# h-brough/TUNA

Hardware: AMD Instinct MI355X
Metric: Fock builds/sec (J+K from the HBM-resident ERI tensor, one density) + SCF wall time (higher is better)
Workload: dtype f64

## Files before the change

tuna_amd/csrc/tf_device.hip:

```cpp
#include <hip/hip_runtime.h>

#include <algorithm>
#include <chrono>
#include <cmath>
#include <cstddef>
#include <cstdio>
#include <cstdlib>
#include <array>
#include <cstring>
#include <condition_variable>
#include <dlfcn.h>
#include <atomic>
#include <map>
#include <memory>
#include <mutex>
#include <thread>
#include <numeric>
#include <string>
#include <vector>

#include "../../include/tunafock.h"
#include "tf_internal.h"
#include "tf_kernels.hip.h"
#include "tf_jkpacked.hip.h"
// ... 2381 lines not shown
    HIPCHK(ctx, e);
    return TF_OK;
}


extern "C++" {
template <int ND>
static int jk_packed_pass(tf_ctx *ctx, hipStream_t st, double *const *dDout, bool cd = false)
{
    const BLayout &L = ctx->bl;
    const int N = ctx->N, NW = L.NW;
    const size_t nn = (size_t)N * N, npr = (size_t)L.NPtot, nrows = (size_t)std::max<long long>(1, ctx->n_rows);
    const tf_ctx::JKTables &T = ctx->jkt[ND - 1];
    const size_t ng = (size_t)std::max(1, T.n_groups);
    JKStrides S{};
    const int MP = ctx->hl.MP;
    S.KS = ctx->hl.KS; S.MP = MP;
    S.planeJd = nrows * NW; S.planeI = ng * N; S.planeJ = nrows * N;
    S.P = nn; S.Pp = npr; S.y = (size_t)T.ypart_len; S.Jd = MP * S.planeJd;
    S.DIc = MP * S.planeI; S.DIr = ng * (size_t)L.RS; S.DJc = MP * S.planeJ; S.DJr = nrows * (size_t)L.RS;
    const size_t per_g = (size_t)N * MP + L.RS;
    double *const pJrow = cd ? ctx->cd_Jrow : ctx->d_Jrow;
    double *const pY = cd ? ctx->cd_ypart + (ND == 2 ? (size_t)std::max<long long>(0, ctx->jkt[0].ypart_len) : 0) : ctx->d_ypart;
    const JKTask *const tasks = cd ? T.d_tasks_cd : T.d_tasks;
    const int n_tasks = cd ? T.n_tasks_cd : T.n_tasks;
    const int *const bucket = cd ? T.bucket_cd : T.bucket;
    double *DI0 = (cd ? ctx->cd_DI : ctx->d_DI) + (ND == 2 ? (size_t)std::max(1, ctx->jkt[0].n_groups) * per_g : 0);
    double *DJ0 = (cd ? ctx->cd_DJ : ctx->d_DJ) + (ND == 2 ? nrows * per_g : 0);
    double *DIc = DI0, *DIr = DI0 + ND * S.DIc, *DJc = DJ0, *DJr = DJ0 + ND * S.DJc;
    if (n_tasks > 0) {
        hipEvent_t ev_after = nullptr;
        if (ctx->prof_jk) {
            if (ctx->prof_used + 2 > ctx->prof_ev.size()) {
                hipEvent_t a, b;
                if (hipEventCreate(&a) == hipSuccess && hipEventCreate(&b) == hipSuccess) { ctx->prof_ev.push_back(a); ctx->prof_ev.push_back(b); }
            }
            if (ctx->prof_used + 2 <= ctx->prof_ev.size()) {
                (void)hipEventRecord(ctx->prof_ev[ctx->prof_used], st);
                ev_after = ctx->prof_ev[ctx->prof_used + 1];
                ctx->prof_used += 2;
            }
        }
        static const bool serial = getenv("TF_JK_SERIAL") != nullptr;
        int n_launch = 0;
        for (int b = 0; b < 3; ++b) n_launch += (bucket[b + 1] > bucket[b] && (TF_JKP_W >> b) >= 1) ? 1 : 0;
        static const int one_launch_below = getenv("TF_JK_ONE_LAUNCH") ? atoi(getenv("TF_JK_ONE_LAUNCH")) : 12000;
        const bool full_supers = T.n_supers > 0 && ctx->n_rows >= 24LL * T.n_supers;
        const bool one_launch = n_launch > 1 && n_tasks < one_launch_below && (ctx->world == 1 || full_supers);
        const bool fork = !serial && !one_launch && ctx->have_streams && n_launch > 1;
        if (fork) (void)hipEventRecord(ctx->sev[0], st);
        int side = 0;
        bool first = true;
        if (one_launch)
            hipLaunchKernelGGL((jk_packed_kernel<ND>), dim3((unsigned)n_tasks), dim3(64 * TF_JKP_W), 0, st, ctx->d_eri, T.d_groups,
                               T.d_supers, tasks, L, L.kinfo, ctx->d_Psym, ctx->d_Pp, pJrow, pY, DIc, DIr, DJc, DJr, S);
        for (int b = 0; b < 3 && !one_launch; ++b) {
            const int t0 = bucket[b], t1 = bucket[b + 1];
            if (!(t1 > t0 && (TF_JKP_W >> b) >= 1)) continue;
            hipStream_t ls = st;
            if (fork && !first) {
                ++side;
                ls = ctx->streams[side];
                (void)hipStreamWaitEvent(ls, ctx->sev[0], 0);
            }
            first = false;
            hipLaunchKernelGGL((jk_packed_kernel<ND>), dim3((unsigned)(t1 - t0)), dim3(64 * (TF_JKP_W >> b)), 0, ls, ctx->d_eri, T.d_groups,
                               T.d_supers, tasks + t0, L, L.kinfo, ctx->d_Psym, ctx->d_Pp, pJrow, pY, DIc, DIr, DJc, DJr, S);
            if (ls != st) {
                (void)hipEventRecord(ctx->sev[side], ls);
                (void)hipStreamWaitEvent(st, ctx->sev[side], 0);
            }
        }
        if (ev_after) (void)hipEventRecord(ev_after, st);
    }
    JKReduce R{};
    R.ypart = pY; R.sy = S.y; R.supers = T.d_supers; R.MC = ctx->hl.MC; R.MP = MP; R.planeI = S.planeI; R.planeJ = S.planeJ; R.nseg = T.nseg; R.jp = T.jp;
    R.Jt = ctx->d_Jt; R.sJt = (size_t)T.nseg * npr;
    R.DIc = DIc; R.sDIc = S.DIc; R.DIr = DIr; R.sDIr = S.DIr; R.DJc = DJc; R.sDJc = S.DJc; R.DJr = DJr; R.sDJr = S.DJr;
    R.gfirst = T.d_gfirst; R.jptr = ctx->d_jptr; R.jrows = ctx->d_jrows; R.row_ij = ctx->d_row_ij; R.xorder = ctx->d_xorder;
    for (int d = 0; d < ND; ++d) R.D[d] = dDout[d];
    { static const int jkr_dbg = getenv("TF_JKR_DBG") ? atoi(getenv("TF_JKR_DBG")) : 0; R.dbg = jkr_dbg; }
    const unsigned nblk = (unsigned)ND * ((unsigned)N * ((N + 127) / 128) + (unsigned)T.jp.bfirst[4] * T.nseg);
    hipLaunchKernelGGL(jk_reduce_kernel, dim3(nblk), dim3(TF_JKR_THREADS), 0, st, R, L);
    return TF_OK;
}
}

static int launch_jk_packed(tf_ctx *ctx, int nd, const double *const *dP, double *const *dJ, double *const *dK, hipStream_t st,
                            const int *nonsym)
{
    const BLayout &L = ctx->bl;
    const int N = ctx->N, NW = L.NW;
    const size_t nn = (size_t)N * N, npr = (size_t)L.NPtot, nrows = (size_t)std::max<long long>(1, ctx->n_rows);
    const dim3 gN((N * N + 255) / 256), b256(256);
    static const bool no_fuse = getenv("TF_JK_NOFUSE") != nullptr;
    bool cd = false;
    {
        static const bool cd_off = getenv("TF_JK_CLASS_DIAGONAL") && getenv("TF_JK_CLASS_DIAGONAL")[0] == '0';
        bool any_general = false;
        for (int d = 0; d < nd; ++d) any_general = any_general || (nonsym && nonsym[d]);
        static const int cd_nmin = getenv("TF_JK_CD_NMIN") ? atoi(getenv("TF_JK_CD_NMIN")) : 160;
        if (ctx->jk_try_class_diagonal && !cd_off && !any_general && N >= cd_nmin && ctx->jkt[0].n_tasks_cd < ctx->jkt[0].n_tasks) {
            if (!ctx->d_cdflag) HIPCHK(ctx, tf_malloc((void **)&ctx->d_cdflag, 2 * sizeof(unsigned long long)));
            cd = true;
            for (int d = 0; d < nd && cd; ++d) {
                HIPCHK(ctx, hipMemsetAsync(ctx->d_cdflag, 0, 2 * sizeof(unsigned long long), st));
                hipLaunchKernelGGL(class_cross_max_kernel, dim3((unsigned)N), dim3(256), 0, st, dP[d], L, ctx->d_cdflag);
                double h[2] = {0.0, 1.0};
                HIPCHK(ctx, hipMemcpyAsync(h, ctx->d_cdflag, sizeof(h), hipMemcpyDeviceToHost, st));
                HIPCHK(ctx, hipStreamSynchronize(st));
                cd = std::isfinite(h[0]) && h[0] < 1e299 && h[1] <= 1e-14 * h[0];
            }
            if (cd && !ctx->cd_Jrow) {
                double **bufs[4] = {&ctx->cd_Jrow, &ctx->cd_ypart, &ctx->cd_DI, &ctx->cd_DJ};
                for (int q = 0; q < 4; ++q) {
                    if (tf_malloc((void **)bufs[q], ctx->cd_bytes[q]) != hipSuccess) {
                        (void)hipGetLastError();
                        for (int u = 0; u < q; ++u) { (void)tf_free(*bufs[u]); *bufs[u] = nullptr; }
                        cd = false;
// ... 901 lines not shown
```

tuna_amd/csrc/tf_jkpacked.hip.h:

```cpp
#pragma once
#include <hip/hip_runtime.h>
#include "tf_layout.hip.h"

#include "tf_packed.h"
#ifndef TF_JKP_OCC4
#define TF_JKP_OCC4 3
#endif
#ifndef TF_JKP_STAGES
#define TF_JKP_STAGES 2
#endif


#ifndef TF_TRI_PAD
#define TF_TRI_PAD 16
#endif
__host__ __device__ inline long long tri_off(long long k)
{
    const long long q = k / TF_TRI_PAD, r = k % TF_TRI_PAD;
    return TF_TRI_PAD * (TF_TRI_PAD * q * (q + 1) / 2 + r * (q + 1));
}
__host__ __device__ inline long long packed_row_len(long long i, long long j) { return (tri_off(i) + j + TF_TRI_PAD) & ~(long long)(TF_TRI_PAD - 1); }

#define TF_JKP_KB 4

__device__ __forceinline__ double ld_stream(const double *p) { return __builtin_nontemporal_load(p); }

__device__ __forceinline__ __amdgpu_buffer_rsrc_t buf_rsrc(const void *base)
{
    return __builtin_amdgcn_make_buffer_rsrc(const_cast<void *>(base), 0, 0x7fffffff, 0x00020000);
}
template <int AUX>
__device__ __forceinline__ double2 buf_load2(__amdgpu_buffer_rsrc_t rs, unsigned lane_off, unsigned uniform_off)
{
    return __builtin_bit_cast(double2, __builtin_amdgcn_raw_buffer_load_b128(rs, (int)lane_off, (int)uniform_off, AUX));
}
template <int AUX>
__device__ __forceinline__ void buf_store2(__amdgpu_buffer_rsrc_t rs, unsigned lane_off, unsigned uniform_off, double2 v)
{
    typedef unsigned u4_t __attribute__((ext_vector_type(4)));
    __builtin_amdgcn_raw_buffer_store_b128(__builtin_bit_cast(u4_t, v), rs, (int)lane_off, (int)uniform_off, AUX);
}

typedef unsigned tf_u2 __attribute__((ext_vector_type(2)));

__device__ __forceinline__ double pair_step32(double a, double b)
{
    const tf_u2 lo = __builtin_amdgcn_permlane32_swap((unsigned)__double2loint(a), (unsigned)__double2loint(b), false, false);
    const tf_u2 hi = __builtin_amdgcn_permlane32_swap((unsigned)__double2hiint(a), (unsigned)__double2hiint(b), false, false);
    return __hiloint2double((int)hi.x, (int)lo.x) + __hiloint2double((int)hi.y, (int)lo.y);
}

__device__ __forceinline__ double pair_step16(double a, double b)
{
    const tf_u2 lo = __builtin_amdgcn_permlane16_swap((unsigned)__double2loint(a), (unsigned)__double2loint(b), false, false);
    const tf_u2 hi = __builtin_amdgcn_permlane16_swap((unsigned)__double2hiint(a), (unsigned)__double2hiint(b), false, false);
    return __hiloint2double((int)hi.x, (int)lo.x) + __hiloint2double((int)hi.y, (int)lo.y);
}

template <int CTRL, int BANK>
__device__ __forceinline__ double dpp_merge(double old, double src)
{
    const int lo = __builtin_amdgcn_update_dpp(__double2loint(old), __double2loint(src), CTRL, 0xF, BANK, false);
    const int hi = __builtin_amdgcn_update_dpp(__double2hiint(old), __double2hiint(src), CTRL, 0xF, BANK, false);
    return __hiloint2double(hi, lo);
}

#define TF_DPP_ROR8 0x128
#define TF_DPP_HALF_MIRROR 0x141
#define TF_DPP_QUAD_IDENT 0xE4
#define TF_DPP_QUAD_XOR1 0xB1
#define TF_DPP_QUAD_XOR2 0x4E

__device__ __forceinline__ double pair_step8(double a, double b)
{
    double recv = dpp_merge<TF_DPP_ROR8, 0x3>(a, a);
    recv = dpp_merge<TF_DPP_ROR8, 0xC>(recv, b);
// ... 97 lines not shown
}
__device__ __forceinline__ double quarter_sum8(const double (&v)[8])
{
    const double w0 = pair_step8(v[0], v[4]), w1 = pair_step8(v[1], v[5]), w2 = pair_step8(v[2], v[6]), w3 = pair_step8(v[3], v[7]);
    const double u0 = pair_step4(w0, w2), u1 = pair_step4(w1, w3);
    double t = pair_step2(u0, u1, (__lane_id() & 2u) != 0u);
    t += dpp_merge<TF_DPP_QUAD_XOR1, 0xF>(t, t);
    return t;
}
__device__ __forceinline__ double quarter_sum1(double t)
{
    t += dpp_merge<TF_DPP_ROR8, 0xF>(t, t);
    return sum8(t);
}
#if TF_JKP_GPW == 4
#define TF_JKP_VSH 1
__device__ __forceinline__ double group_sum8(const double (&v)[8]) { return quarter_sum8(v); }
__device__ __forceinline__ double group_sum1(double t) { return quarter_sum1(t); }
__device__ __forceinline__ double across_groups(double t) { t = pair_step32(t, t); return pair_step16(t, t); }
#else
#define TF_JKP_VSH 2
__device__ __forceinline__ double group_sum8(const double (&v)[8]) { return half_sum8(v); }
__device__ __forceinline__ double group_sum1(double t) { return half_sum1(t); }
__device__ __forceinline__ double across_groups(double t) { return pair_step32(t, t); }
#endif
#define TF_JKP_VMASK ((1 << TF_JKP_VSH) - 1)

#define TF_BUF_OOB 0x80000000u
template <int AUX>
__device__ __forceinline__ void buf_store1(__amdgpu_buffer_rsrc_t rs, unsigned lane_off, unsigned uniform_off, double v)
{
    typedef unsigned u2_t __attribute__((ext_vector_type(2)));
    __builtin_amdgcn_raw_buffer_store_b64(__builtin_bit_cast(u2_t, v), rs, (int)lane_off, (int)uniform_off, AUX);
}
template <int AUX>
__device__ __forceinline__ double buf_load1(__amdgpu_buffer_rsrc_t rs, unsigned lane_off, unsigned uniform_off)
{
    return __builtin_bit_cast(double, __builtin_amdgcn_raw_buffer_load_b64(rs, (int)lane_off, (int)uniform_off, AUX));
}

struct JKWave {
    const double *Tb, *X, *Pp;
    const KInfo *kinfo;
    long long NPtot;
    int N, i;
    int kI0, c0, lam0, width, cm;
    int sec;
    __amdgpu_buffer_rsrc_t rt;
    int rp;
    double *yg, *DIr, *DJr;
    size_t RS, ystride, dstrideI, dstrideJ;
};

template <int ND>
struct JKLane {
    int h, q, lam, lI;
    int nr, lamj0, r0, g;
    unsigned xrow;
    unsigned gb, unr, p0;
    unsigned djoff, dioff;
    double ppij[JKShape<ND>::VR];
    double2 pil[ND], pjl[JKShape<ND>::VR];
    double2 colI[ND], colJ[JKShape<ND>::VR];
};

enum { JKP_DIAG = 1, JKP_FULL = 2 };

template <int ND>
struct JKLoad { double2 m[JKShape<ND>::RB], pp[ND]; int cnt; };

template <int ND, bool ALLR, int MODE>
__device__ __forceinline__ void jkp_load(JKLoad<ND> &L, const JKLane<ND> &C, const JKWave &U, int kap)
{
    constexpr int RB = JKShape<ND>::RB;
    const KInfo ki = U.kinfo[kap];
    const int pc = (ki.cnt + TF_SEG_PAD - 1) & ~(TF_SEG_PAD - 1);
    L.cnt = ki.cnt;
    const bool v = (MODE == JKP_FULL) || C.lam < ki.cnt;
    const __amdgpu_buffer_rsrc_t rt = U.rt;
    const unsigned seg = __umul24(C.p0, (unsigned)pc) + __umul24(C.unr, (unsigned)(U.sec + ki.offA)) + C.gb;
    const unsigned dsel = 8u * seg;
#ifdef TF_ABL_ALLVALID
    const unsigned voff = 16u * (unsigned)C.q + dsel;
#define TF_ABL_ROWOK(r) true
#else
    const unsigned voff = v ? 16u * (unsigned)C.q + dsel : TF_BUF_OOB;
#define TF_ABL_ROWOK(r) (ALLR || (r) < C.nr)
#endif
#pragma unroll
#ifdef TF_ABL_NOTENSOR
    for (int r = 0; r < RB; ++r) L.m[r] = make_double2(C.ppij[r] + (double)kap, C.ppij[r] - (double)voff);
#else
    for (int r = 0; r < RB; ++r) L.m[r] = buf_load2<2>(rt, TF_ABL_ROWOK(r) ? voff : TF_BUF_OOB, 8u * (unsigned)(r * pc));
#endif
    const long long bk = (long long)ki.offA + U.lam0;
#pragma unroll
    for (int d = 0; d < ND; ++d) L.pp[d] = buf_load2<0>(buf_rsrc(U.Pp + d * U.NPtot + bk), v ? 16u * (unsigned)C.q : TF_BUF_OOB, 0u);
}

template <int ND>
__device__ __forceinline__ void jkp_row1(const JKLane<ND> &C, const JKLoad<ND> &L, double (&jd)[JKShape<ND>::VR],
                                         double (&rJ)[JKShape<ND>::VR], double (&rI)[ND], double2 (&jt)[ND])
{
    constexpr int RB = JKShape<ND>::RB;
#pragma unroll
    for (int d = 0; d < ND; ++d) {
        jt[d] = make_double2(0.0, 0.0);
        rI[d] = 0.0;
#pragma unroll
        for (int r = 0; r < RB; ++r) {
            const int v = d * RB + r;
            const double2 m = L.m[r];
            jd[v] += m.x * L.pp[d].x + m.y * L.pp[d].y;
            jt[d].x += m.x * C.ppij[v]; jt[d].y += m.y * C.ppij[v];
            const double2 pj = C.pjl[v];
            rI[d] += m.x * pj.x + m.y * pj.y;
            rJ[v] = m.x * C.pil[d].x + m.y * C.pil[d].y;
        }
    }
}

template <int ND, int MODE>
__device__ __forceinline__ void jkp_row2(JKLane<ND> &C, const JKLoad<ND> &L, const JKWave &U, const double (&pjk)[JKShape<ND>::VR], const double (&pik)[ND])
{
    constexpr int RB = JKShape<ND>::RB;
    const int lim = L.cnt - U.cm;
    const double o0 = (MODE == JKP_FULL || C.lam < lim) ? 1.0 : 0.0, o1 = (MODE == JKP_FULL || C.lam + 1 < lim) ? 1.0 : 0.0;
#pragma unroll
    for (int r = 0; r < RB; ++r) {
        const double mx = (MODE == JKP_FULL) ? L.m[r].x : L.m[r].x * o0, my = (MODE == JKP_FULL) ? L.m[r].y : L.m[r].y * o1;
#pragma unroll
        for (int d = 0; d < ND; ++d) {
            const int v = d * RB + r;
            C.colI[d].x += mx * pjk[v]; C.colI[d].y += my * pjk[v];
            C.colJ[v].x += mx * pik[d]; C.colJ[v].y += my * pik[d];
        }
    }
}

template <int ND, bool ALLR>
__device__ __forceinline__ void jkp_p_k(const JKLane<ND> &C, const JKWave &U, int kI, double (&pjk)[JKShape<ND>::VR], double (&pik)[ND])
{
    constexpr int RB = JKShape<ND>::RB;
#pragma unroll
    for (int d = 0; d < ND; ++d) {
        const double *Pd = U.X + (size_t)d * U.N * U.N;
        const __amdgpu_buffer_rsrc_t rx = buf_rsrc(Pd);
#pragma unroll
#ifdef TF_ABL_NOPJK
        for (int r = 0; r < RB; ++r) pjk[d * RB + r] = C.ppij[d * RB + r];
#else
        for (int r = 0; r < RB; ++r) pjk[d * RB + r] = buf_load1<0>(rx, (ALLR || r < C.nr) ? C.xrow : TF_BUF_OOB, 8u * (unsigned)(r * U.N + kI));
#endif
        pik[d] = Pd[(size_t)U.i * U.N + kI];
    }
}

template <int ND>
__device__ __forceinline__ void jkp_last(JKLane<ND> &C, const JKWave &U, const double (&pjk)[JKShape<ND>::VR], const double (&pik)[ND],
                                         double (&jd)[JKShape<ND>::VR], double (&rJ)[JKShape<ND>::VR], double (&rI)[ND], double2 (&jt2)[ND])
{
    constexpr int RB = JKShape<ND>::RB;
    const int i = U.i, lamlast = C.lamj0 + C.nr - 1;
    const KInfo kiL = U.kinfo[i - U.kI0];
    const long long bk = kiL.offA;
    const int pc = (kiL.cnt + TF_SEG_PAD - 1) & ~(TF_SEG_PAD - 1);
    const double *Tk = U.Tb + ((long long)C.gb + (long long)C.unr * (U.sec + kiL.offA) + (long long)C.p0 * pc);
#pragma unroll
    for (int d = 0; d < ND; ++d) { rI[d] = 0.0; jt2[d] = make_double2(0.0, 0.0); }
#pragma unroll
    for (int v = 0; v < JKShape<ND>::VR; ++v) rJ[v] = 0.0;
#pragma unroll
    for (int e = 0; e < 2; ++e) {
        const int lam = C.lam + e;
        const bool valid = lam <= lamlast;
        double mrow[RB];
#pragma unroll
        for (int r = 0; r < RB; ++r) mrow[r] = (r < C.nr && lam <= C.lamj0 + r) ? ld_stream(Tk + r * pc + lam) : 0.0;
#pragma unroll
        for (int d = 0; d < ND; ++d) {
            const double pp = valid ? U.Pp[d * U.NPtot + bk + lam] : 0.0;
            const double pil = e ? C.pil[d].y : C.pil[d].x;
            double jt = 0.0, cI = 0.0;
#pragma unroll
            for (int r = 0; r < RB; ++r) {
                const int v = d * RB + r;
                const double mr = mrow[r];
                const bool diag = (lam == C.lamj0 + r);
                jd[v] += mr * pp;
                jt += diag ? 0.0 : mr * C.ppij[v];
                const double mk = diag ? 0.5 * mr : mr;
                rI[d] += mk * (e ? C.pjl[v].y : C.pjl[v].x);
                rJ[v] += mk * pil;
                const double mc = (C.lI + e != i) ? mk : 0.0;
                cI += mc * pjk[v];
                if (e) C.colJ[v].y += mc * pik[d]; else C.colJ[v].x += mc * pik[d];
            }
            if (e) { C.colI[d].y += cI; jt2[d].y = jt; } else { C.colI[d].x += cI; jt2[d].x = jt; }
        }
    }
}

template <int ND, bool ALLR>
__device__ __forceinline__ void jkp_row_sums(const JKLane<ND> &C, const JKWave &U, int kap, double (&rJ)[JKShape<ND>::VR], const double (&rI)[ND])
{
    constexpr int VR = JKShape<ND>::VR, RB = JKShape<ND>::RB;
    const int v = (C.q >> TF_JKP_VSH) & 7;
    const bool first = (C.q & TF_JKP_VMASK) == 0;
    if constexpr (VR == 8) {
        const double tJ = group_sum8(rJ);
        const int d = v / RB, r = v - d * RB;
        buf_store1<0>(buf_rsrc(U.DJr + kap), (first && r < C.nr) ? C.djoff + 8u * (unsigned)(d * U.dstrideJ + (size_t)r * U.RS) : TF_BUF_OOB, 0u, tJ);
#pragma unroll
        for (int dd = 0; dd < ND; ++dd) {
            const double tI = group_sum1(rI[dd]);
            buf_store1<0>(buf_rsrc(U.DIr + dd * U.dstrideI + kap), (C.q == 0 && C.nr > 0) ? C.dioff : TF_BUF_OOB, 0u, tI);
        }
    } else {
        static_assert(ND == 1 && VR == 4, "shapes: 8 virtual rows, or 4 rows of one density");
        const double vals[8] = {rJ[0], rJ[1], rJ[2], rJ[3], rI[0], 0.0, 0.0, 0.0};
        const double t = group_sum8(vals);
        buf_store1<0>(buf_rsrc(U.DJr + kap), (first && v < C.nr) ? C.djoff + 8u * (unsigned)((size_t)v * U.RS) : TF_BUF_OOB, 0u, t);
        buf_store1<0>(buf_rsrc(U.DIr + kap), (first && v == 4 && C.nr > 0) ? C.dioff : TF_BUF_OOB, 0u, t);
    }
}

__device__ __forceinline__ void jkp_lds_barrier() { asm volatile("s_waitcnt lgkmcnt(0)\n\ts_barrier" ::: "memory"); }

template <int ND, int MODE>
__device__ __forceinline__ void jkp_merge_jt(const JKWave &U, double2 *slots, int nw, int w, int lane, int kb, int k1)
{
    jkp_lds_barrier();
    const int nwg = (int)(blockDim.x >> 6);
    for (int kk = w; kk < TF_JKP_KB; kk += nwg) {
        const int kap = kb + kk;
        if (kap >= k1) break;
        const KInfo ki = U.kinfo[kap];
#pragma unroll
        for (int d = 0; d < ND; ++d) {
            double2 t = slots[((kk * TF_JKP_W) * ND + d) * 64 + lane];
            for (int u = 1; u < nw; ++u) { const double2 x = slots[((kk * TF_JKP_W + u) * ND + d) * 64 + lane]; t.x += x.x; t.y += x.y; }
            t.x = across_groups(t.x); t.y = across_groups(t.y);
            if (lane < TF_JKP_LG && (MODE == JKP_FULL || U.lam0 + 2 * lane < ki.cnt))
                buf_store2<2>(buf_rsrc(U.yg + d * U.ystride + ki.offA + U.lam0), 16u * (unsigned)lane, 0u, t);
        }
    }
    jkp_lds_barrier();
}


template <int ND, bool ALLR, int MODE>
__device__ __forceinline__ void jkp_segment(const JKWave &U, JKLane<ND> &C, double (&jd)[JKShape<ND>::VR], int k0, int k1, int lane, bool active,
                                            double2 *slots, int nw, int w)
{
    constexpr int JBB = JKShape<ND>::VR, S = TF_JKP_STAGES;
    static_assert(TF_JKP_KB % S == 0, "the ring position of a step must be a compile-time constant");
    if (k0 >= k1) return;
    JKLoad<ND> R[S];
    if (active) {
#pragma unroll
        for (int s = 0; s < S - 1; ++s) jkp_load<ND, ALLR, MODE>(R[s], C, U, min(k0 + s, k1 - 1));
    }
    for (int kb = k0; kb < k1; kb += TF_JKP_KB) {
        if (active) {
#pragma unroll
            for (int kk = 0; kk < TF_JKP_KB; ++kk) {
                const int k = kb + kk;
                if (k < k1) {
                    double pjk[JBB], pik[ND], rJ[JBB], rI[ND];
                    double2 jt[ND];
                    jkp_p_k<ND, ALLR>(C, U, U.kI0 + k, pjk, pik);
                    jkp_load<ND, ALLR, MODE>(R[(kk + S - 1) % S], C, U, min(k + S - 1, k1 - 1));
#ifdef TF_ABL_LOADSONLY
                    {
#pragma unroll
                        for (int r = 0; r < JBB / ND; ++r) jd[r] += R[kk % S].m[r].x + R[kk % S].m[r].y;
                        jd[0] += R[kk % S].pp[0].x + pjk[0] + pik[0];
                    }
                    continue;
#endif
                    jkp_row1<ND>(C, R[kk % S], jd, rJ, rI, jt);
#ifdef TF_ABL_NOMERGE
                    {
                        const KInfo ki = U.kinfo[k];
#pragma unroll
                        for (int d = 0; d < ND; ++d) {
                            double2 t = jt[d];
                            t.x = across_groups(t.x); t.y = across_groups(t.y);
                            buf_store2<2>(buf_rsrc(U.yg + d * U.ystride + ki.offA + U.lam0), (lane < TF_JKP_LG && (MODE == JKP_FULL || U.lam0 + 2 * lane < ki.cnt)) ? 16u * (unsigned)lane : TF_BUF_OOB, 0u, t);
                        }
                    }
#else
#pragma unroll
                    for (int d = 0; d < ND; ++d) slots[((kk * TF_JKP_W + w) * ND + d) * 64 + lane] = jt[d];
#endif
                    jkp_row_sums<ND, ALLR>(C, U, k, rJ, rI);
                    jkp_row2<ND, MODE>(C, R[kk % S], U, pjk, pik);
                }
            }
        }
#ifndef TF_ABL_NOMERGE
        jkp_merge_jt<ND, MODE>(U, slots, nw, w, lane, kb, k1);
#endif
    }
}

template <int ND, bool ALLR>
__device__ __forceinline__ void jkp_task(const JKWave &U, JKLane<ND> &C, int NW, int wchunk, int lane, bool active, double2 *slots, int nw,
                                         int w, int kap0, int kd1, int klim, bool last, double *__restrict__ Jd, size_t strideJd,
                                         double *__restrict__ DIc, size_t strideDIc, double *__restrict__ DJc, size_t strideDJc)
{
    constexpr int JBB = JKShape<ND>::VR, RB = JBB / ND;
    const int N = U.N, i = U.i;
    const bool in0 = 2 * C.q < U.width, in1 = 2 * C.q + 1 < U.width;
    {
#pragma unroll
        for (int d = 0; d < ND; ++d) {
            const double *Pd = U.X + (size_t)d * N * N;
            const double *Pi = Pd + (size_t)i * N;
            C.pil[d] = make_double2(in0 ? Pi[C.lI] : 0.0, in1 ? Pi[C.lI + 1] : 0.0);
            C.colI[d] = make_double2(0.0, 0.0);
#pragma unroll
            for (int r = 0; r < RB; ++r) {
                const bool have = r < C.nr;
                const double *Pj = Pd + (C.xrow >> 3) + (size_t)r * N;
                C.pjl[d * RB + r] = make_double2((in0 && have) ? Pj[C.lI] : 0.0, (in1 && have) ? Pj[C.lI + 1] : 0.0);
                C.colJ[d * RB + r] = make_double2(0.0, 0.0);
            }
        }
    }
    double jd[JBB];
#pragma unroll
    for (int v = 0; v < JBB; ++v) jd[v] = 0.0;

    jkp_segment<ND, ALLR, JKP_DIAG>(U, C, jd, kap0, kd1, lane, active, slots, nw, w);
    jkp_segment<ND, ALLR, JKP_FULL>(U, C, jd, kd1, klim, lane, active, slots, nw, w);
    if (last) {
        double2 jt[ND];
#pragma unroll
        for (int d = 0; d < ND; ++d) jt[d] = make_double2(0.0, 0.0);
        if (active) {
            double pjk[JBB], pik[ND], rJ[JBB], rI[ND];
            jkp_p_k<ND, false>(C, U, i, pjk, pik);
            jkp_last<ND>(C, U, pjk, pik, jd, rJ, rI, jt);
            jkp_row_sums<ND, ALLR>(C, U, i - U.kI0, rJ, rI);
        }
#pragma unroll
        for (int d = 0; d < ND; ++d) slots[(w * ND + d) * 64 + lane] = jt[d];
        __syncthreads();
        if (w == 0) {
            const KInfo ki = U.kinfo[i - U.kI0];
#pragma unroll
            for (int d = 0; d < ND; ++d) {
                double2 t = slots[d * 64 + lane];
                for (int u = 1; u < nw; ++u) { const double2 x = slots[(u * ND + d) * 64 + lane]; t.x += x.x; t.y += x.y; }
                t.x = across_groups(t.x); t.y = across_groups(t.y);
                if (lane < TF_JKP_LG && U.lam0 + 2 * lane < ki.cnt) buf_store2<2>(buf_rsrc(U.yg + d * U.ystride + ki.offA + U.lam0), 16u * (unsigned)lane, 0u, t);
            }
        }
    }
    if (!active) return;
#pragma unroll
    for (int e = 0; e < 2; ++e) {
        if ((e ? in1 : in0) && C.nr > 0) {
            const int l = C.lI + e;
#pragma unroll
            for (int d = 0; d < ND; ++d) {
                DIc[d * strideDIc + (size_t)C.g * N + l] = e ? C.colI[d].y : C.colI[d].x;
#pragma unroll
                for (int r = 0; r < RB; ++r)
                    if (r < C.nr) DJc[d * strideDJc + (size_t)(C.r0 + r) * N + l] = e ? C.colJ[d * RB + r].y : C.colJ[d * RB + r].x;
            }
        }
    }
    {
        double vals[8];
#pragma unroll
        for (int v = 0; v < 8; ++v) vals[v] = v < JBB ? jd[v < JBB ? v : 0] : 0.0;
        const double t = group_sum8(vals);
        const int v = (C.q >> TF_JKP_VSH) & 7, d = v / RB, r = v - d * RB;
        if ((C.q & TF_JKP_VMASK) == 0 && v < JBB && r < C.nr) Jd[d * strideJd + (size_t)(C.r0 + r) * NW + wchunk] = t;
    }
}

struct JKStrides { size_t P, Pp, y, Jd, DIc, DIr, DJc, DJr;
                   size_t planeJd, planeI, planeJ; int KS, MP; };

template <int ND>
__global__ __launch_bounds__(64 * TF_JKP_W, TF_JKP_STAGES > 2 ? 1 : (JKShape<ND>::VR == 4 ? TF_JKP_OCC4 : 2)) void jk_packed_kernel(const double *__restrict__ T, const JKGroup *__restrict__ groups,
                                                                  const JKSuper *__restrict__ supers,
                                                                  const JKTask *__restrict__ tasks, BLayout L,
                                                                  const KInfo *__restrict__ kinfo ,
                                                                  const double *__restrict__ X, const double *__restrict__ Pp,
                                                                  double *__restrict__ Jd, double *__restrict__ ypart,
                                                                  double *__restrict__ DIc, double *__restrict__ DIr,
                                                                  double *__restrict__ DJc, double *__restrict__ DJr, JKStrides S)
{
    constexpr int JBB = JKShape<ND>::VR, RB = JBB / ND;
    __shared__ double2 slots[TF_JKP_KB * TF_JKP_W * ND * 64];
    const JKTask t = tasks[blockIdx.x];
    const JKSuper sg = supers[t.super];
    const int w = __builtin_amdgcn_readfirstlane(threadIdx.x >> 6), lane = threadIdx.x & 63;
    constexpr int GPW = TF_JKP_GPW;
    const int nw = (sg.ng + GPW - 1) / GPW;
    const bool active = w < nw;
    int ids[GPW], ngw = 0;
#pragma unroll
    for (int g = 0; g < GPW; ++g) {
        const int gi = sg.g0 + (active ? GPW * w : 0) + g;
        const bool have = active && GPW * w + g < sg.ng;
        ids[g] = have ? gi : sg.g0 + (active ? GPW * w : 0);
        ngw += have ? 1 : 0;
    }
    {
        auto below = [&](int x, int y) {
            const long long ux = groups[x].ub, uy = groups[y].ub;
            return ux < uy || (ux == uy && groups[x].p0 < groups[y].p0);
        };
        int lowest = 0;
#pragma unroll
        for (int g = 1; g < GPW; ++g) if (g < ngw && below(ids[g], ids[lowest])) lowest = g;
        const int tswap = ids[0]; ids[0] = ids[lowest]; ids[lowest] = tswap;
#pragma unroll
        for (int g = 0; g < GPW; ++g) ids[g] = __builtin_amdgcn_readfirstlane(ids[g]);
    }
    const JKGroup gA = groups[ids[0]];
    const int N = L.N, NW = L.NW, c = sg.c;
    const int b = L.chunk_cls[t.w], a = b ^ c;
    JKWave U;
    U.N = N; U.i = __builtin_amdgcn_readfirstlane(gA.i);
    U.kI0 = bl_cstart(L, a); U.c0 = L.chunk_c0[t.w]; U.lam0 = U.c0 - bl_cstart(L, b); U.width = L.chunk_width[t.w]; U.cm = (c == 0) ? 1 : 0;
    U.sec = groups[ids[0]].secoff[a];
    U.Tb = T + gA.ub; U.X = X; U.NPtot = (long long)S.Pp;
    U.rt = buf_rsrc(U.Tb + U.lam0);
    const long long pbase = bl_cbase(L, c) + bl_fullsec(L, c, a);
    U.Pp = Pp + pbase;
    U.kinfo = kinfo + (size_t)c * N + U.kI0;
    U.yg = ypart + sg.yoff + bl_fullsec(L, c, a); U.ystride = S.y;
    U.RS = (size_t)L.RS;
    U.rp = L.rpoff[c * NW + t.w];
    JKLane<ND> C;
    C.h = lane / TF_JKP_LG; C.q = lane % TF_JKP_LG;
    C.lam = U.lam0 + 2 * C.q; C.lI = U.c0 + 2 * C.q;
    int gmin = ids[0], rmin = gA.r0;
    C.nr = active ? gA.nr : 0; C.lamj0 = gA.lamj0; C.r0 = gA.r0; C.g = ids[0];
    C.gb = 0u; C.unr = (unsigned)gA.unr; C.p0 = (unsigned)gA.p0;
    int j0 = gA.j0;
    bool all_full = active && gA.nr == RB;
#pragma unroll
    for (int g = 1; g < GPW; ++g) {
        const JKGroup gG = groups[ids[g]];
        const bool have = g < ngw;
        gmin = min(gmin, ids[g]); rmin = min(rmin, gG.r0);
        all_full = all_full && have && gG.nr == RB;
        if (C.h == g) {
            C.nr = have ? gG.nr : 0; C.lamj0 = gG.lamj0; C.r0 = gG.r0; C.g = ids[g]; j0 = gG.j0;
            C.gb = (unsigned)(gG.ub - gA.ub); C.unr = (unsigned)gG.unr; C.p0 = (unsigned)gG.p0;
        }
    }
    U.DIr = DIr + (size_t)gmin * L.RS + U.rp; U.dstrideI = S.DIr;
    U.DJr = DJr + (size_t)rmin * L.RS + U.rp; U.dstrideJ = S.DJr;
    C.xrow = 8u * (unsigned)(j0 * N);
    C.dioff = 8u * (unsigned)((C.g - gmin) * L.RS);
    C.djoff = 8u * (unsigned)((C.r0 - rmin) * L.RS);
    {
        const int ci = L.clsI[gA.i];
        const long long pij = bl_cbase(L, c) + bl_fullsec(L, c, ci) + kinfo[(size_t)c * N + gA.i].offA + C.lamj0;
#pragma unroll
        for (int d = 0; d < ND; ++d)
#pragma unroll
            for (int r = 0; r < RB; ++r) C.ppij[d * RB + r] = (r < C.nr) ? Pp[d * S.Pp + pij + r] : 0.0;
    }
    const int kap00 = L.kap0[c * NW + t.w], ke = supers[t.super].ke[a];
    const int kap0 = kap00 + t.part * S.KS, kend = min(ke, kap0 + S.KS);
    const bool last = (a == L.clsI[gA.i]) && kend == ke;
    const int klim = kend - (last ? 1 : 0);
    const int kd1 = min(max(L.kapF[c * NW + t.w], kap0), klim);
    Jd += (size_t)t.part * S.planeJd; DIc += (size_t)t.part * S.planeI; DJc += (size_t)t.part * S.planeJ;
    if (all_full)
        jkp_task<ND, true>(U, C, NW, t.w, lane, active, slots, nw, w, kap0, kd1, klim, last, Jd, S.Jd, DIc, S.DIc, DJc, S.DJc);
    else
        jkp_task<ND, false>(U, C, NW, t.w, lane, active, slots, nw, w, kap0, kd1, klim, last, Jd, S.Jd, DIc, S.DIc, DJc, S.DJc);
}

__device__ __forceinline__ void jt_reduce_block(int bx, int by, int nseg, const double *__restrict__ ypart, const JKSuper *__restrict__ supers,
                                                const JKJtPlan &JP, const BLayout &L, double *__restrict__ out)
{
    int c = 0;
    while (c < 3 && bx >= JP.bfirst[c + 1]) ++c;
    const long long q = (long long)(bx - JP.bfirst[c]) * TF_JKR_THREADS + threadIdx.x;
    if (q >= bl_np(L, c)) return;
    const int kI = L.gk[bl_gbase(L, c) + (int)(q / TF_SEG_PAD)];
    const int a = L.clsI[kI], kap = kI - bl_cstart(L, a);
    const KInfo ki = L.kinfo[(size_t)c * L.N + kI];
    double s = 0.0;
    if ((int)(q - bl_fullsec(L, c, a)) - ki.offA < ki.cnt) {
        const int n = JP.sfirst[c + 1] - JP.sfirst[c], per = (n + nseg - 1) / nseg;
        const int s0 = JP.sfirst[c] + by * per, s1 = min(JP.sfirst[c + 1], s0 + per);
        for (int g = s0; g < s1; ++g) {
            if (supers[g].ke[a] <= kap) break;
            s += ypart[supers[g].yoff + q];
        }
    }
    out[(size_t)by * L.NPtot + bl_cbase(L, c) + q] = s;
}

#ifndef TF_JKR_U
#define TF_JKR_U 2
#endif
#ifndef TF_JKR_MCMAX
#define TF_JKR_MCMAX 4
#endif
struct KdLoads { double2 c, s[TF_JKR_MCMAX]; };
__device__ __forceinline__ void kd_issue(KdLoads &q, const double *__restrict__ colp, const double *__restrict__ rowp, int N, int MC, int y, bool two, bool on)
{
    const double2 z = make_double2(0.0, 0.0);
    q.c = !on ? z : (two ? *reinterpret_cast<const double2 *>(colp + y) : make_double2(colp[y], 0.0));
#pragma unroll
    for (int sl = 0; sl < TF_JKR_MCMAX; ++sl)
        q.s[sl] = !(on && sl < MC) ? z : (two ? *reinterpret_cast<const double2 *>(rowp + (size_t)sl * N + y) : make_double2(rowp[(size_t)sl * N + y], 0.0));
}
__device__ __forceinline__ double2 kd_sum(const KdLoads &q, const double *__restrict__ rowp, int N, int MC, int y, bool two, bool on)
{
    double2 t = q.c;
#pragma unroll
    for (int sl = 0; sl < TF_JKR_MCMAX; ++sl) { t.x += q.s[sl].x; t.y += q.s[sl].y; }
    for (int sl = TF_JKR_MCMAX; sl < MC && on; ++sl) {
        const double2 v = two ? *reinterpret_cast<const double2 *>(rowp + (size_t)sl * N + y) : make_double2(rowp[(size_t)sl * N + y], 0.0);
        t.x += v.x; t.y += v.y;
    }
    return t;
}
__device__ __forceinline__ double2 kd_vec(const double *__restrict__ colp, const double *__restrict__ rowp, int N, int MC, int y, bool two)
{
    double2 t = two ? *reinterpret_cast<const double2 *>(colp + y) : make_double2(colp[y], 0.0);
// ... 298 lines not shown
```

Baseline: 432.4.

## Hoist per-task buffer descriptors and prefetch kinfo ahead in one-density JK kernel

```diff
diff --git a/tuna_amd/csrc/tf_device.hip b/tuna_amd/csrc/tf_device.hip
--- a/tuna_amd/csrc/tf_device.hip
+++ b/tuna_amd/csrc/tf_device.hip
@@ -2457,7 +2457,7 @@
         int side = 0;
         bool first = true;
         if (one_launch)
-            hipLaunchKernelGGL((jk_packed_kernel<ND>), dim3((unsigned)n_tasks), dim3(64 * TF_JKP_W), 0, st, ctx->d_eri, T.d_groups,
+            hipLaunchKernelGGL((jk_packed_kernel<ND, JKRing<ND>::S>), dim3((unsigned)n_tasks), dim3(64 * TF_JKP_W), 0, st, ctx->d_eri, T.d_groups,
                                T.d_supers, tasks, L, L.kinfo, ctx->d_Psym, ctx->d_Pp, pJrow, pY, DIc, DIr, DJc, DJr, S);
         for (int b = 0; b < 3 && !one_launch; ++b) {
             const int t0 = bucket[b], t1 = bucket[b + 1];
@@ -2469,7 +2469,7 @@
                 (void)hipStreamWaitEvent(ls, ctx->sev[0], 0);
             }
             first = false;
-            hipLaunchKernelGGL((jk_packed_kernel<ND>), dim3((unsigned)(t1 - t0)), dim3(64 * (TF_JKP_W >> b)), 0, ls, ctx->d_eri, T.d_groups,
+            hipLaunchKernelGGL((jk_packed_kernel<ND, JKRing<ND>::S>), dim3((unsigned)(t1 - t0)), dim3(64 * (TF_JKP_W >> b)), 0, ls, ctx->d_eri, T.d_groups,
                                T.d_supers, tasks + t0, L, L.kinfo, ctx->d_Psym, ctx->d_Pp, pJrow, pY, DIc, DIr, DJc, DJr, S);
             if (ls != st) {
                 (void)hipEventRecord(ctx->sev[side], ls);
diff --git a/tuna_amd/csrc/tf_jkpacked.hip.h b/tuna_amd/csrc/tf_jkpacked.hip.h
--- a/tuna_amd/csrc/tf_jkpacked.hip.h
+++ b/tuna_amd/csrc/tf_jkpacked.hip.h
@@ -9,6 +9,12 @@
 #ifndef TF_JKP_STAGES
 #define TF_JKP_STAGES 2
 #endif
+#ifndef TF_JKP_PRING
+#define TF_JKP_PRING (TF_JKP_STAGES > 2)
+#endif
+template <int ND> struct JKRing { static constexpr int S = ND == 1 ? TF_JKP_STAGES : 2; };
+template <int ND, int S> struct JKRingP { static constexpr bool PR = ND == 1 && (TF_JKP_PRING) != 0; };
+template <int ND> struct JKStep { static constexpr bool HOIST = ND == 1; };
 
 
 #ifndef TF_TRI_PAD
@@ -22,6 +28,10 @@
 __host__ __device__ inline long long packed_row_len(long long i, long long j) { return (tri_off(i) + j + TF_TRI_PAD) & ~(long long)(TF_TRI_PAD - 1); }
 
 #define TF_JKP_KB 4
+#ifndef TF_JKP_KB1
+#define TF_JKP_KB1 TF_JKP_KB
+#endif
+constexpr int jkp_kb(int nd, int stages) { return nd != 1 ? TF_JKP_KB : (TF_JKP_KB1 % stages == 0 ? TF_JKP_KB1 : 2 * stages); }
 
 __device__ __forceinline__ double ld_stream(const double *p) { return __builtin_nontemporal_load(p); }
 
@@ -225,6 +235,8 @@
     size_t RS, ystride, dstrideI, dstrideJ;
 };
 
+struct JKDesc { __amdgpu_buffer_rsrc_t rpp, rdj, rdi, ry; };
+
 template <int ND>
 struct JKLane {
     int h, q, lam, lI;
@@ -241,6 +253,26 @@
 
 template <int ND>
 struct JKLoad { double2 m[JKShape<ND>::RB], pp[ND]; int cnt; };
+template <int ND>
+struct JKLoadR { JKLoad<ND> t; double pjk[JKShape<ND>::VR], pik[ND]; };
+
+template <int ND, bool ALLR>
+__device__ __forceinline__ void jkp_p_k(const JKLane<ND> &C, const JKWave &U, int kI, double (&pjk)[JKShape<ND>::VR], double (&pik)[ND])
+{
+    constexpr int RB = JKShape<ND>::RB;
+#pragma unroll
+    for (int d = 0; d < ND; ++d) {
+        const double *Pd = U.X + (size_t)d * U.N * U.N;
+        const __amdgpu_buffer_rsrc_t rx = buf_rsrc(Pd);
+#pragma unroll
+#ifdef TF_ABL_NOPJK
+        for (int r = 0; r < RB; ++r) pjk[d * RB + r] = C.ppij[d * RB + r];
+#else
+        for (int r = 0; r < RB; ++r) pjk[d * RB + r] = buf_load1<0>(rx, (ALLR || r < C.nr) ? C.xrow : TF_BUF_OOB, 8u * (unsigned)(r * U.N + kI));
+#endif
+        pik[d] = Pd[(size_t)U.i * U.N + kI];
+    }
+}
 
 template <int ND, bool ALLR, int MODE>
 __device__ __forceinline__ void jkp_load(JKLoad<ND> &L, const JKLane<ND> &C, const JKWave &U, int kap)
@@ -271,6 +303,40 @@
     for (int d = 0; d < ND; ++d) L.pp[d] = buf_load2<0>(buf_rsrc(U.Pp + d * U.NPtot + bk), v ? 16u * (unsigned)C.q : TF_BUF_OOB, 0u);
 }
 
+template <int ND, bool ALLR, int MODE, bool PR>
+__device__ __forceinline__ void jkp_load_ahead(JKLoadR<ND> &L, const JKLane<ND> &C, const JKWave &U, const JKDesc &Q, const KInfo ki, int kap)
+{
+    constexpr int RB = JKShape<ND>::RB;
+    static_assert(ND == 1, "the two-density kernel keeps jkp_load");
+    const int offA = __builtin_amdgcn_readfirstlane(ki.offA), cnt = __builtin_amdgcn_readfirstlane(ki.cnt);
+    if constexpr (PR) {
+#pragma unroll
+#ifdef TF_ABL_NOPJK
+        for (int r = 0; r < RB; ++r) L.pjk[r] = C.ppij[r];
+#else
+        for (int r = 0; r < RB; ++r) L.pjk[r] = buf_load1<0>(buf_rsrc(U.X), (ALLR || r < C.nr) ? C.xrow : TF_BUF_OOB, 8u * (unsigned)(r * U.N + U.kI0 + kap));
+#endif
+    }
+    const int pc = (cnt + TF_SEG_PAD - 1) & ~(TF_SEG_PAD - 1);
+    L.t.cnt = cnt;
+    const bool v = (MODE == JKP_FULL) || C.lam < cnt;
+    const unsigned seg = __umul24(C.p0, (unsigned)pc) + __umul24(C.unr, (unsigned)(U.sec + offA)) + C.gb;
+    const unsigned dsel = 8u * seg;
+#ifdef TF_ABL_ALLVALID
+    const unsigned voff = 16u * (unsigned)C.q + dsel;
+#else
+    const unsigned voff = v ? 16u * (unsigned)C.q + dsel : TF_BUF_OOB;
+#endif
+#pragma unroll
+#ifdef TF_ABL_NOTENSOR
+    for (int r = 0; r < RB; ++r) L.t.m[r] = make_double2(C.ppij[r] + (double)kap, C.ppij[r] - (double)voff);
+#else
+    for (int r = 0; r < RB; ++r) L.t.m[r] = buf_load2<2>(U.rt, TF_ABL_ROWOK(r) ? voff : TF_BUF_OOB, 8u * (unsigned)(r * pc));
+#endif
+    L.t.pp[0] = buf_load2<0>(Q.rpp, v ? 16u * (unsigned)C.q : TF_BUF_OOB, 8u * (unsigned)offA);
+    if constexpr (PR) L.pik[0] = U.X[(size_t)U.i * U.N + U.kI0 + kap];
+}
+
 template <int ND>
 __device__ __forceinline__ void jkp_row1(const JKLane<ND> &C, const JKLoad<ND> &L, double (&jd)[JKShape<ND>::VR],
                                          double (&rJ)[JKShape<ND>::VR], double (&rI)[ND], double2 (&jt)[ND])
@@ -308,24 +374,6 @@
             C.colI[d].x += mx * pjk[v]; C.colI[d].y += my * pjk[v];
             C.colJ[v].x += mx * pik[d]; C.colJ[v].y += my * pik[d];
         }
-    }
-}
-
-template <int ND, bool ALLR>
-__device__ __forceinline__ void jkp_p_k(const JKLane<ND> &C, const JKWave &U, int kI, double (&pjk)[JKShape<ND>::VR], double (&pik)[ND])
-{
-    constexpr int RB = JKShape<ND>::RB;
-#pragma unroll
-    for (int d = 0; d < ND; ++d) {
-        const double *Pd = U.X + (size_t)d * U.N * U.N;
-        const __amdgpu_buffer_rsrc_t rx = buf_rsrc(Pd);
-#pragma unroll
-#ifdef TF_ABL_NOPJK
-        for (int r = 0; r < RB; ++r) pjk[d * RB + r] = C.ppij[d * RB + r];
-#else
-        for (int r = 0; r < RB; ++r) pjk[d * RB + r] = buf_load1<0>(rx, (ALLR || r < C.nr) ? C.xrow : TF_BUF_OOB, 8u * (unsigned)(r * U.N + kI));
-#endif
-        pik[d] = Pd[(size_t)U.i * U.N + kI];
     }
 }
 
@@ -375,12 +423,12 @@
 }
 
 template <int ND, bool ALLR>
-__device__ __forceinline__ void jkp_row_sums(const JKLane<ND> &C, const JKWave &U, int kap, double (&rJ)[JKShape<ND>::VR], const double (&rI)[ND])
+__device__ __forceinline__ void jkp_row_sums(const JKLane<ND> &C, const JKWave &U, const JKDesc &Q, int kap, double (&rJ)[JKShape<ND>::VR], const double (&rI)[ND])
 {
     constexpr int VR = JKShape<ND>::VR, RB = JKShape<ND>::RB;
     const int v = (C.q >> TF_JKP_VSH) & 7;
     const bool first = (C.q & TF_JKP_VMASK) == 0;
-    if constexpr (VR == 8) {
+    if constexpr (VR == 8 && !JKStep<ND>::HOIST) {
         const double tJ = group_sum8(rJ);
         const int d = v / RB, r = v - d * RB;
         buf_store1<0>(buf_rsrc(U.DJr + kap), (first && r < C.nr) ? C.djoff + 8u * (unsigned)(d * U.dstrideJ + (size_t)r * U.RS) : TF_BUF_OOB, 0u, tJ);
@@ -389,23 +437,29 @@
             const double tI = group_sum1(rI[dd]);
             buf_store1<0>(buf_rsrc(U.DIr + dd * U.dstrideI + kap), (C.q == 0 && C.nr > 0) ? C.dioff : TF_BUF_OOB, 0u, tI);
         }
+    } else if constexpr (VR == 8) {
+        static_assert(ND == 1, "descriptors per task: the one-density kernel");
+        const double tJ = group_sum8(rJ);
+        buf_store1<0>(Q.rdj, (first && v < C.nr) ? C.djoff + 8u * (unsigned)((size_t)v * U.RS) : TF_BUF_OOB, 8u * (unsigned)kap, tJ);
+        const double tI = group_sum1(rI[0]);
+        buf_store1<0>(Q.rdi, (C.q == 0 && C.nr > 0) ? C.dioff : TF_BUF_OOB, 8u * (unsigned)kap, tI);
     } else {
         static_assert(ND == 1 && VR == 4, "shapes: 8 virtual rows, or 4 rows of one density");
         const double vals[8] = {rJ[0], rJ[1], rJ[2], rJ[3], rI[0], 0.0, 0.0, 0.0};
         const double t = group_sum8(vals);
-        buf_store1<0>(buf_rsrc(U.DJr + kap), (first && v < C.nr) ? C.djoff + 8u * (unsigned)((size_t)v * U.RS) : TF_BUF_OOB, 0u, t);
-        buf_store1<0>(buf_rsrc(U.DIr + kap), (first && v == 4 && C.nr > 0) ? C.dioff : TF_BUF_OOB, 0u, t);
+        buf_store1<0>(Q.rdj, (first && v < C.nr) ? C.djoff + 8u * (unsigned)((size_t)v * U.RS) : TF_BUF_OOB, 8u * (unsigned)kap, t);
+        buf_store1<0>(Q.rdi, (first && v == 4 && C.nr > 0) ? C.dioff : TF_BUF_OOB, 8u * (unsigned)kap, t);
     }
 }
 
 __device__ __forceinline__ void jkp_lds_barrier() { asm volatile("s_waitcnt lgkmcnt(0)\n\ts_barrier" ::: "memory"); }
 
-template <int ND, int MODE>
-__device__ __forceinline__ void jkp_merge_jt(const JKWave &U, double2 *slots, int nw, int w, int lane, int kb, int k1)
+template <int ND, int KB, int MODE>
+__device__ __forceinline__ void jkp_merge_jt(const JKWave &U, const JKDesc &Q, double2 *slots, int nw, int w, int lane, int kb, int k1)
 {
     jkp_lds_barrier();
     const int nwg = (int)(blockDim.x >> 6);
-    for (int kk = w; kk < TF_JKP_KB; kk += nwg) {
+    for (int kk = w; kk < KB; kk += nwg) {
         const int kap = kb + kk;
         if (kap >= k1) break;
         const KInfo ki = U.kinfo[kap];
@@ -414,45 +468,62 @@
             double2 t = slots[((kk * TF_JKP_W) * ND + d) * 64 + lane];
             for (int u = 1; u < nw; ++u) { const double2 x = slots[((kk * TF_JKP_W + u) * ND + d) * 64 + lane]; t.x += x.x; t.y += x.y; }
             t.x = across_groups(t.x); t.y = across_groups(t.y);
-            if (lane < TF_JKP_LG && (MODE == JKP_FULL || U.lam0 + 2 * lane < ki.cnt))
-                buf_store2<2>(buf_rsrc(U.yg + d * U.ystride + ki.offA + U.lam0), 16u * (unsigned)lane, 0u, t);
+            if (lane < TF_JKP_LG && (MODE == JKP_FULL || U.lam0 + 2 * lane < ki.cnt)) {
+                if constexpr (JKStep<ND>::HOIST) buf_store2<2>(Q.ry, 16u * (unsigned)lane, 8u * (unsigned)ki.offA, t);
+                else buf_store2<2>(buf_rsrc(U.yg + d * U.ystride + ki.offA + U.lam0), 16u * (unsigned)lane, 0u, t);
+            }
         }
     }
     jkp_lds_barrier();
 }
 
-
-template <int ND, bool ALLR, int MODE>
-__device__ __forceinline__ void jkp_segment(const JKWave &U, JKLane<ND> &C, double (&jd)[JKShape<ND>::VR], int k0, int k1, int lane, bool active,
-                                            double2 *slots, int nw, int w)
-{
-    constexpr int JBB = JKShape<ND>::VR, S = TF_JKP_STAGES;
-    static_assert(TF_JKP_KB % S == 0, "the ring position of a step must be a compile-time constant");
+template <int ND> __device__ __forceinline__ JKLoad<ND> &jkp_slot(JKLoad<ND> &x) { return x; }
+template <int ND> __device__ __forceinline__ JKLoad<ND> &jkp_slot(JKLoadR<ND> &x) { return x.t; }
+
+template <int ND, int S, bool ALLR, int MODE>
+__device__ __forceinline__ void jkp_segment(const JKWave &U, const JKDesc &Q, JKLane<ND> &C, double (&jd)[JKShape<ND>::VR], int k0, int k1, int lane,
+                                            bool active, double2 *slots, int nw, int w)
+{
+    constexpr int JBB = JKShape<ND>::VR, KB = jkp_kb(ND, S);
+    constexpr bool H = JKStep<ND>::HOIST, PR = H && JKRingP<ND, S>::PR;
+    static_assert(S >= 2 && KB % S == 0, "the ring position of a step must be a compile-time constant");
     if (k0 >= k1) return;
-    JKLoad<ND> R[S];
+    typename std::conditional<H, JKLoadR<ND>, JKLoad<ND>>::type R[S];
+    [[maybe_unused]] KInfo kn = {0, 0};
     if (active) {
 #pragma unroll
-        for (int s = 0; s < S - 1; ++s) jkp_load<ND, ALLR, MODE>(R[s], C, U, min(k0 + s, k1 - 1));
-    }
-    for (int kb = k0; kb < k1; kb += TF_JKP_KB) {
+        for (int s = 0; s < S - 1; ++s) {
+            if constexpr (H) { const int kl = min(k0 + s, k1 - 1); jkp_load_ahead<ND, ALLR, MODE, PR>(R[s], C, U, Q, U.kinfo[kl], kl); }
+            else jkp_load<ND, ALLR, MODE>(R[s], C, U, min(k0 + s, k1 - 1));
+        }
+        if constexpr (H) kn = U.kinfo[min(k0 + S - 1, k1 - 1)];
+    }
+    for (int kb = k0; kb < k1; kb += KB) {
         if (active) {
 #pragma unroll
-            for (int kk = 0; kk < TF_JKP_KB; ++kk) {
+            for (int kk = 0; kk < KB; ++kk) {
                 const int k = kb + kk;
                 if (k < k1) {
                     double pjk[JBB], pik[ND], rJ[JBB], rI[ND];
                     double2 jt[ND];
-                    jkp_p_k<ND, ALLR>(C, U, U.kI0 + k, pjk, pik);
-                    jkp_load<ND, ALLR, MODE>(R[(kk + S - 1) % S], C, U, min(k + S - 1, k1 - 1));
+                    if constexpr (!PR) jkp_p_k<ND, ALLR>(C, U, U.kI0 + k, pjk, pik);
+                    if constexpr (H) {
+                        const KInfo kc = kn;
+                        kn = U.kinfo[min(k + S, k1 - 1)];
+                        jkp_load_ahead<ND, ALLR, MODE, PR>(R[(kk + S - 1) % S], C, U, Q, kc, min(k + S - 1, k1 - 1));
+                    } else
+                        jkp_load<ND, ALLR, MODE>(R[(kk + S - 1) % S], C, U, min(k + S - 1, k1 - 1));
 #ifdef TF_ABL_LOADSONLY
                     {
 #pragma unroll
-                        for (int r = 0; r < JBB / ND; ++r) jd[r] += R[kk % S].m[r].x + R[kk % S].m[r].y;
-                        jd[0] += R[kk % S].pp[0].x + pjk[0] + pik[0];
+                        for (int r = 0; r < JBB / ND; ++r) jd[r] += jkp_slot<ND>(R[kk % S]).m[r].x + jkp_slot<ND>(R[kk % S]).m[r].y;
+                        jd[0] += jkp_slot<ND>(R[kk % S]).pp[0].x;
+                        if constexpr (PR) jd[0] += R[kk % S].pjk[0] + R[kk % S].pik[0];
+                        else jd[0] += pjk[0] + pik[0];
                     }
                     continue;
 #endif
-                    jkp_row1<ND>(C, R[kk % S], jd, rJ, rI, jt);
+                    jkp_row1<ND>(C, jkp_slot<ND>(R[kk % S]), jd, rJ, rI, jt);
 #ifdef TF_ABL_NOMERGE
                     {
                         const KInfo ki = U.kinfo[k];
@@ -467,19 +538,20 @@
 #pragma unroll
                     for (int d = 0; d < ND; ++d) slots[((kk * TF_JKP_W + w) * ND + d) * 64 + lane] = jt[d];
 #endif
-                    jkp_row_sums<ND, ALLR>(C, U, k, rJ, rI);
-                    jkp_row2<ND, MODE>(C, R[kk % S], U, pjk, pik);
+                    jkp_row_sums<ND, ALLR>(C, U, Q, k, rJ, rI);
+                    if constexpr (PR) jkp_row2<ND, MODE>(C, R[kk % S].t, U, R[kk % S].pjk, R[kk % S].pik);
+                    else jkp_row2<ND, MODE>(C, jkp_slot<ND>(R[kk % S]), U, pjk, pik);
                 }
             }
         }
 #ifndef TF_ABL_NOMERGE
-        jkp_merge_jt<ND, MODE>(U, slots, nw, w, lane, kb, k1);
-#endif
-    }
-}
-
-template <int ND, bool ALLR>
-__device__ __forceinline__ void jkp_task(const JKWave &U, JKLane<ND> &C, int NW, int wchunk, int lane, bool active, double2 *slots, int nw,
+        jkp_merge_jt<ND, KB, MODE>(U, Q, slots, nw, w, lane, kb, k1);
+#endif
+    }
+}
+
+template <int ND, int S, bool ALLR>
+__device__ __forceinline__ void jkp_task(const JKWave &U, const JKDesc &Q, JKLane<ND> &C, int NW, int wchunk, int lane, bool active, double2 *slots, int nw,
                                          int w, int kap0, int kd1, int klim, bool last, double *__restrict__ Jd, size_t strideJd,
                                          double *__restrict__ DIc, size_t strideDIc, double *__restrict__ DJc, size_t strideDJc)
 {
@@ -506,8 +578,8 @@
 #pragma unroll
     for (int v = 0; v < JBB; ++v) jd[v] = 0.0;
 
-    jkp_segment<ND, ALLR, JKP_DIAG>(U, C, jd, kap0, kd1, lane, active, slots, nw, w);
-    jkp_segment<ND, ALLR, JKP_FULL>(U, C, jd, kd1, klim, lane, active, slots, nw, w);
+    jkp_segment<ND, S, ALLR, JKP_DIAG>(U, Q, C, jd, kap0, kd1, lane, active, slots, nw, w);
+    jkp_segment<ND, S, ALLR, JKP_FULL>(U, Q, C, jd, kd1, klim, lane, active, slots, nw, w);
     if (last) {
         double2 jt[ND];
 #pragma unroll
@@ -516,7 +588,7 @@
             double pjk[JBB], pik[ND], rJ[JBB], rI[ND];
             jkp_p_k<ND, false>(C, U, i, pjk, pik);
             jkp_last<ND>(C, U, pjk, pik, jd, rJ, rI, jt);
-            jkp_row_sums<ND, ALLR>(C, U, i - U.kI0, rJ, rI);
+            jkp_row_sums<ND, ALLR>(C, U, Q, i - U.kI0, rJ, rI);
         }
 #pragma unroll
         for (int d = 0; d < ND; ++d) slots[(w * ND + d) * 64 + lane] = jt[d];
@@ -559,8 +631,8 @@
 struct JKStrides { size_t P, Pp, y, Jd, DIc, DIr, DJc, DJr;
                    size_t planeJd, planeI, planeJ; int KS, MP; };
 
-template <int ND>
-__global__ __launch_bounds__(64 * TF_JKP_W, TF_JKP_STAGES > 2 ? 1 : (JKShape<ND>::VR == 4 ? TF_JKP_OCC4 : 2)) void jk_packed_kernel(const double *__restrict__ T, const JKGroup *__restrict__ groups,
+template <int ND, int STG>
+__global__ __launch_bounds__(64 * TF_JKP_W, (JKShape<ND>::VR == 4 && STG == 2) ? TF_JKP_OCC4 : 2) void jk_packed_kernel(const double *__restrict__ T, const JKGroup *__restrict__ groups,
                                                                   const JKSuper *__restrict__ supers,
                                                                   const JKTask *__restrict__ tasks, BLayout L,
                                                                   const KInfo *__restrict__ kinfo ,
@@ -570,7 +642,7 @@
                                                                   double *__restrict__ DJc, double *__restrict__ DJr, JKStrides S)
 {
     constexpr int JBB = JKShape<ND>::VR, RB = JBB / ND;
-    __shared__ double2 slots[TF_JKP_KB * TF_JKP_W * ND * 64];
+    __shared__ double2 slots[jkp_kb(ND, STG) * TF_JKP_W * ND * 64];
     const JKTask t = tasks[blockIdx.x];
     const JKSuper sg = supers[t.super];
     const int w = __builtin_amdgcn_readfirstlane(threadIdx.x >> 6), lane = threadIdx.x & 63;
@@ -633,6 +705,8 @@
     }
     U.DIr = DIr + (size_t)gmin * L.RS + U.rp; U.dstrideI = S.DIr;
     U.DJr = DJr + (size_t)rmin * L.RS + U.rp; U.dstrideJ = S.DJr;
+    JKDesc Q;
+    if constexpr (JKStep<ND>::HOIST) { Q.rpp = buf_rsrc(U.Pp + U.lam0); Q.ry = buf_rsrc(U.yg + U.lam0); Q.rdj = buf_rsrc(U.DJr); Q.rdi = buf_rsrc(U.DIr); }
     C.xrow = 8u * (unsigned)(j0 * N);
     C.dioff = 8u * (unsigned)((C.g - gmin) * L.RS);
     C.djoff = 8u * (unsigned)((C.r0 - rmin) * L.RS);
@@ -651,9 +725,9 @@
     const int kd1 = min(max(L.kapF[c * NW + t.w], kap0), klim);
     Jd += (size_t)t.part * S.planeJd; DIc += (size_t)t.part * S.planeI; DJc += (size_t)t.part * S.planeJ;
     if (all_full)
-        jkp_task<ND, true>(U, C, NW, t.w, lane, active, slots, nw, w, kap0, kd1, klim, last, Jd, S.Jd, DIc, S.DIc, DJc, S.DJc);
+        jkp_task<ND, STG, true>(U, Q, C, NW, t.w, lane, active, slots, nw, w, kap0, kd1, klim, last, Jd, S.Jd, DIc, S.DIc, DJc, S.DJc);
     else
-        jkp_task<ND, false>(U, C, NW, t.w, lane, active, slots, nw, w, kap0, kd1, klim, last, Jd, S.Jd, DIc, S.DIc, DJc, S.DJc);
+        jkp_task<ND, STG, false>(U, Q, C, NW, t.w, lane, active, slots, nw, w, kap0, kd1, klim, last, Jd, S.Jd, DIc, S.DIc, DJc, S.DJc);
 }
 
 __device__ __forceinline__ void jt_reduce_block(int bx, int by, int nseg, const double *__restrict__ ypart, const JKSuper *__restrict__ supers,
```

Result: no change. 431.1 (-0.3%).
